# JacekNaruniec/LiveScan3D

Hardware: AMD Instinct MI355X
Metric: fused frames/s (N x 512x424 depth -> merged cloud) (higher is better)
Workload: dtype f32

## Files before the change

### livescan3d_amd/csrc/fusion.hip

```cpp


#include "fusion_shared.hpp"

namespace {

struct Iv { float lo, hi; };
__device__ __forceinline__ Iv iv_scale(Iv a, float c) { const float x = a.lo * c, y = a.hi * c; return c >= 0.0f ? Iv{x, y} : Iv{y, x}; }
__device__ __forceinline__ Iv iv_shift(Iv a, float c) { return Iv{a.lo + c, a.hi + c}; }
__device__ __forceinline__ Iv iv_sum(Iv a, Iv b) { return Iv{a.lo + b.lo, a.hi + b.hi}; }
__device__ __forceinline__ bool iv_finite(Iv a) { return isfinite(a.lo) && isfinite(a.hi); }

__device__ __forceinline__ float depth_to_metres1(float d)
{
    const f2 z = depth_to_metres2(f2{d, d});
    return z.x;
}

__device__ __forceinline__ int classify_range(int a, int b, float xfac, float yfac, const SensorParams &P, const float (&bx)[6])
{
    if (a == b) {
        f2 ox, oy, oz;
        unproject2(f2{(float)a, (float)a}, f2{xfac, xfac}, f2{yfac, yfac}, P, ox, oy, oz);
        const bool rejected = (ox.x < bx[0]) | (ox.x > bx[3]) | (oy.x < bx[1]) | (oy.x > bx[4]) | (oz.x < bx[2]) | (oz.x > bx[5]);
        return rejected ? 0 : 1;
// ... 116 lines not shown
#pragma unroll
        for (int i = 0; i < kTickGroup; i++) {
            const int wt = wave_count_thr(in[i], lo, cnt);
            if (lane == 0) s_cnt[wave][i] = wt;
        }
    } else {
        const SensorParams P = a.params[t.f];
        float xf[kPxPerLane], yf[kPxPerLane];
        tile_factors<VEC>(t, xf, yf);
#pragma unroll 1
        for (int i = 0; i < nt; i++) {
            Tile ti = t;
            ti.dptr = t.dptr + (long long)i * a.tick_depth_stride;
            Inputs ix;
            load_inputs<VEC, false>(ti, ix);
            bool keep[kPxPerLane];
            uint4 unused[kPxPerLane];
            compute_pixels<false>(a, P, ix, xf, yf, keep, unused);
            int wt = 0;
#pragma unroll
            for (int k = 0; k < kPxPerLane; k++) wt += __popcll(__ballot(keep[k]));
            if (lane == 0) s_cnt[wave][i] = wt;
        }
    }
    __syncthreads();
    if ((int)threadIdx.x < nt)
        a.tile_counts[(long long)(tick0 + threadIdx.x) * a.tiles_per_tick + tile] =
            s_cnt[0][threadIdx.x] + s_cnt[1][threadIdx.x] + s_cnt[2][threadIdx.x] + s_cnt[3][threadIdx.x];
}

constexpr unsigned long long kFlagAggregate = 1ull << 62;
constexpr unsigned long long kFlagPrefix = 2ull << 62;
constexpr int kSpinLimit = 1 << 20;

constexpr int kEpochShift = 34;
constexpr unsigned long long kTileAggregate = 1ull << 32, kTilePrefix = 2ull << 32;

__device__ __forceinline__ int tile_lookback(const FuseArgs &a, int tick, int tile, int tile_tot, int lane)
{
    unsigned long long *st = a.run_state + (long long)tick * a.tiles_per_tick;
    const unsigned long long tag = (unsigned long long)a.epoch << kEpochShift;
    if (lane == 0)
        __hip_atomic_store(&st[tile], tag | (tile == 0 ? kTilePrefix : kTileAggregate) | (unsigned int)tile_tot, __ATOMIC_RELAXED,
                           __HIP_MEMORY_SCOPE_AGENT);
    int acc = 0;
    int pos = tile - 1 - lane;
    bool done = tile == 0;
    int spins = 0;
    const bool near_polls = a.n_ticks > 1;
    while (!done) {
        unsigned long long w = tag | kTilePrefix;
        if (pos >= 0) {
            if (near_polls && (spins & 3) != 3) w = __hip_atomic_load(&st[pos], __ATOMIC_RELAXED, __HIP_MEMORY_SCOPE_WORKGROUP);
            else w = __hip_atomic_load(&st[pos], __ATOMIC_RELAXED, __HIP_MEMORY_SCOPE_AGENT);
        }
        bool again = false;
        const unsigned int flag = (w >> kEpochShift) == a.epoch ? (unsigned int)(w >> 32) & 3u : 0u;
        const unsigned long long pref = __ballot(flag == 2);
        const int first = pref ? __ffsll((long long)pref) - 1 : 63;
        const unsigned long long relevant = first >= 63 ? ~0ull : ((2ull << first) - 1ull);
        const bool poisoned = (__ballot(flag == 3) & relevant) != 0;
        if (poisoned || (__ballot(flag == 0) & relevant) != 0) {
            if (poisoned || ++spins > kSpinLimit) {
                if (lane == 0) {
                    atomicExch(a.error_flag, 1);
                    if (a.offsets_mirror) a.offsets_mirror[a.n_frames + 1] = 1;
                    __hip_atomic_store(&st[tile], tag | (3ull << 32), __ATOMIC_RELAXED, __HIP_MEMORY_SCOPE_AGENT);
                }
                return -1;
            }
            __builtin_amdgcn_s_sleep(1);
            again = true;
        } else {
            acc += wave_sum(lane <= first ? (int)(unsigned int)w : 0);
            if (pref) done = true;
        }
        if (!done && !again) pos -= 64;
    }
    if (lane == 0 && tile != 0)
        __hip_atomic_store(&st[tile], tag | kTilePrefix | (unsigned int)(acc + tile_tot), __ATOMIC_RELAXED, __HIP_MEMORY_SCOPE_AGENT);
    return acc;
}


template <int MODE, bool VEC, bool LAZY = false, bool HOST = false>
__global__ __launch_bounds__(kThreads) void fuse_kernel(const FuseArgs a)
{
    constexpr bool kWrite = MODE != 0;
    __shared__ uint4 stage[kWrite ? kStageSlots : 1];
    __shared__ int s_wave_tot[4];
    __shared__ int s_wave_next[4];
    __shared__ int s_base;
    const int lane = threadIdx.x & 63;
    const int wave = threadIdx.x >> 6;
    int tick = blockIdx.x / a.tiles_per_tick;
    int tile = blockIdx.x - tick * a.tiles_per_tick;
    if (kWrite && a.chunk > 0) {
        const int per_chunk = a.chunk * a.n_ticks;
        const int chunk = blockIdx.x / per_chunk;
        const int r = blockIdx.x - chunk * per_chunk;
        const int width = min(a.chunk, a.tiles_per_tick - chunk * a.chunk);
        tick = r / width;
        tile = chunk * a.chunk + (r - tick * width);
    }
    tile += a.tile0;
    if (MODE == 1 && a.reverse_ticks) tick = a.n_ticks - 1 - tick;
    const int lin = tick * a.tiles_per_tick + tile;

    const Tile t = locate(a, tick, tile);
    Inputs in;
    load_inputs<VEC, kWrite && !LAZY>(t, in);
    Inputs nx;
    if (MODE == 3) {
        Tile tn = t;
        tn.dptr = a.depth_next + tick * a.tick_depth_stride + t.pix_base;
        load_inputs<VEC, false>(tn, nx);
    }
    const SensorParams P = a.params[t.f];
    float xf[kPxPerLane], yf[kPxPerLane];
    tile_factors<VEC>(t, xf, yf);
    bool keep[kPxPerLane];
    uint4 vert[kPxPerLane];
    compute_pixels<kWrite>(a, P, in, xf, yf, keep, vert);
    if (kWrite && LAZY) {
        bool any = false;
#pragma unroll
        for (int k = 0; k < kPxPerLane; k++) any |= keep[k];
        if (any) {
            load_rgb<VEC>(t, in);
#pragma unroll
            for (int k = 0; k < kPxPerLane; k++) vert[k].x = rgba_of(in, k);
        }
    }
    if (MODE == 3) {
        int wt = 0;
        bool arithmetic = true;
        if (a.thr) {
            unsigned int lo[kPxPerLane], cnt[kPxPerLane];
            bool any_flagged;
            load_thresholds<VEC>(a, t, lo, cnt, any_flagged);
            arithmetic = any_flagged;
            if (!any_flagged) wt = wave_count_thr(nx, lo, cnt);
        }
        if (arithmetic) {
            bool keep_n[kPxPerLane];
            uint4 unused[kPxPerLane];
            compute_pixels<false>(a, P, nx, xf, yf, keep_n, unused);
#pragma unroll
            for (int k = 0; k < kPxPerLane; k++) wt += __popcll(__ballot(keep_n[k]));
        }
        if (lane == 0) s_wave_next[wave] = wt;
    }

    int below, wave_total;
    rank_from_masks(keep, below, wave_total);
    if (lane == 0) s_wave_tot[wave] = wave_total;
    int base = 0, counted = 0;
    if (MODE == 1 || MODE == 3) {
        base = a.tile_counts[lin];
        counted = (tile + 1 < a.tiles_per_tick ? a.tile_counts[lin + 1] : a.offsets[tick * (a.n_frames + 1) + a.n_frames]) - base;
    }
    __syncthreads();
    int wave_off = 0, tile_tot = 0;
#pragma unroll
    for (int i = 0; i < 4; i++) {
        const int v = s_wave_tot[i];
        if (i < wave) wave_off += v;
        tile_tot += v;
    }
    if (MODE == 0) {
        if (threadIdx.x == 0) a.tile_counts[lin] = tile_tot;
        return;
    }
    if (MODE == 3 && threadIdx.x == 0) a.tile_counts_next[lin] = s_wave_next[0] + s_wave_next[1] + s_wave_next[2] + s_wave_next[3];
    if (MODE == 4) {
        if (wave == 0) {
            const int b = tile_lookback(a, tick, tile, tile_tot, lane);
            if (lane == 0) s_base = b;
        }
        __syncthreads();
        base = s_base;
        if (base < 0) {
            if (threadIdx.x == 0 && tile == a.tiles_per_tick - 1) {
                a.offsets[tick * (a.n_frames + 1) + a.n_frames] = -1;
                if (a.offsets_mirror) a.offsets_mirror[a.n_frames] = -1;
            }
            return;
        }
        if (threadIdx.x == 0) {
            int *off = a.offsets + tick * (a.n_frames + 1);
            if (t.frame_start) off[t.f] = base;
            if (tile == a.tiles_per_tick - 1) off[a.n_frames] = base + tile_tot;
            if (a.offsets_mirror) {
                if (t.frame_start) a.offsets_mirror[t.f] = base;
                if (tile == a.tiles_per_tick - 1) a.offsets_mirror[a.n_frames] = base + tile_tot;
            }
            if (a.group_end_mirror && blockIdx.x == gridDim.x - 1) *a.group_end_mirror = base + tile_tot;
        }
    }
    if (MODE != 4 && tile_tot != counted) {
        if (threadIdx.x == 0) atomicExch(a.error_flag, 2);
        return;
    }
    if (VEC ? a.pm_first != nullptr : a.pixmap != nullptr) {
        const int p0 = t.px0 + threadIdx.x * kPxPerLane;
        if (p0 < t.npix) {
            int r = base + wave_off + below;
            if (VEC) {
                unsigned int m = 0;
#pragma unroll
                for (int k = 0; k < kPxPerLane; k++) m |= keep[k] ? (1u << k) : 0u;
                const long long g = (tick * a.tick_depth_stride + t.pix_base + p0) >> 3;
                a.pm_first[g] = r;
                a.pm_mask[g] = (unsigned char)m;
            } else {
                int *pm = a.pixmap + tick * a.tick_depth_stride + t.pix_base + p0;
#pragma unroll
                for (int k = 0; k < kPxPerLane; k++) {
                    if (p0 + k < t.npix) pm[k] = keep[k] ? r : -1;
                    r += keep[k] ? 1 : 0;
                }
            }
        }
    }
    stage_and_store(stage, keep, vert, wave_off + below, tile_tot, a.out + tick * a.tick_vert_stride + base, HOST || (MODE == 4 && a.host_out != 0));
}



template <bool VEC>
__global__ __launch_bounds__(kThreads) void run_kernel(const FuseArgs a)
{
    __shared__ uint4 stage[kStageSlots];
    __shared__ int s_wave_tot[4];
    __shared__ int s_run;
    __shared__ int s_base;
    const int lane = threadIdx.x & 63;
    const int wave = threadIdx.x >> 6;

    const int tick = blockIdx.x % a.n_ticks;
    if (threadIdx.x == 0) s_run = (int)atomicAdd(a.ticket + 32 * tick, 1u);
    __syncthreads();
    const int run = s_run;
    if (run >= a.runs_per_tick) return;
    const int t0 = run * a.tiles_per_run;
    const int t1 = min(t0 + a.tiles_per_run, a.tiles_per_tick);

    int wave_total = 0;
    {
        Tile t = locate(a, tick, t0);
        Inputs in;
        load_inputs<VEC, false>(t, in);
        for (int tile = t0; tile < t1; tile++) {
            Tile tn = t;
            Inputs nx = in;
            if (tile + 1 < t1) {
                tn = locate(a, tick, tile + 1);
                load_inputs<VEC, false>(tn, nx);
            }
            bool counted = false;
            if (a.thr) {
                unsigned int lo[kPxPerLane], cnt[kPxPerLane];
                bool any_flagged;
                load_thresholds<VEC>(a, t, lo, cnt, any_flagged);
                if (!any_flagged) {
                    wave_total += wave_count_thr(in, lo, cnt);
                    counted = true;
                }
            }
            if (!counted) {
                bool keep[kPxPerLane];
                uint4 unused[kPxPerLane];
                compute_tile<VEC, false>(a, t, in, keep, unused);
#pragma unroll
                for (int k = 0; k < kPxPerLane; k++) wave_total += __popcll(__ballot(keep[k]));
            }
            t = tn;
            in = nx;
        }
    }
    if (lane == 0) s_wave_tot[wave] = wave_total;
    __syncthreads();
    const int run_tot = s_wave_tot[0] + s_wave_tot[1] + s_wave_tot[2] + s_wave_tot[3];
// ... 30 lines not shown
            }
            const int v = (lane <= first) ? (int)(unsigned int)w : 0;
            acc += wave_sum(v);
            if (pref) done = true;
            else pos -= 64;
        }
        if (lane == 0) {
            if (run != 0) {
                const unsigned long long w = kFlagPrefix | (unsigned int)(acc + run_tot);
                __hip_atomic_store(&st[run], w, __ATOMIC_RELAXED, __HIP_MEMORY_SCOPE_AGENT);
            }
            s_base = acc;
        }
    }
    __syncthreads();
    int running = s_base;

    int *off = a.offsets + (long long)tick * (a.n_frames + 1);
    for (int tile = t0; tile < t1; tile++) {
        Tile tn = t;
        Inputs nx = in;
        if (tile + 1 < t1) {
            tn = locate(a, tick, tile + 1);
            load_inputs<VEC, true>(tn, nx);
        }
        bool keep[kPxPerLane];
        uint4 vert[kPxPerLane];
        compute_tile<VEC, true>(a, t, in, keep, vert);
        int below, wave_tot2;
        rank_from_masks(keep, below, wave_tot2);
        if (lane == 0) s_wave_tot[wave] = wave_tot2;
        __syncthreads();
        int wave_off = 0, tile_tot = 0;
#pragma unroll
        for (int i = 0; i < 4; i++) {
            const int v = s_wave_tot[i];
            if (i < wave) wave_off += v;
            tile_tot += v;
        }
        if (threadIdx.x == 0 && t.frame_start) off[t.f] = running;
        if (tile_tot > 0) {
            stage_and_store(stage, keep, vert, wave_off + below, tile_tot, a.out + tick * a.tick_vert_stride + running);
        } else {
            __syncthreads();
        }
        running += tile_tot;
        t = tn;
        in = nx;
    }
    if (threadIdx.x == 0 && t1 == a.tiles_per_tick) off[a.n_frames] = running;
}


__global__ __launch_bounds__(kThreads) void table_kernel(const FrameDesc *frames, const SensorParams *params, int n_frames, float *xtab,
                                                         float *ytab)
{
    const int f = blockIdx.y;
    if (f >= n_frames) return;
    const FrameDesc fd = frames[f];
    const SensorParams P = params[f];
    for (int i = blockIdx.x * kThreads + threadIdx.x; i < fd.w + fd.h; i += gridDim.x * kThreads) {
        if (i < fd.w) xtab[fd.xtab_off + i] = ((float)i - P.cx) / P.fx;
        else ytab[fd.ytab_off + (i - fd.w)] = (P.cy - (float)(i - fd.w)) / P.fy;
    }
}

}


extern "C" LsnFusion * lsnFusionCreate(int device, int n_ticks, int n_maps, const int *widths, const int *heights)
{
    return lsn::guarded("lsnFusionCreate", static_cast<LsnFusion *>(nullptr), [&]() -> LsnFusion * {
        lsn::clear_error();
        if (n_ticks <= 0 || n_maps <= 0 || !widths || !heights) {
            lsn::set_error("lsnFusionCreate: bad arguments (n_ticks=%d n_maps=%d)", n_ticks, n_maps);
            return nullptr;
        }
        LSN_HIP_NULL(hipSetDevice(device));
        LsnFusion *p = new (std::nothrow) LsnFusion();
        if (!p) return nullptr;
        p->device = device;
        if (const char *env = getenv("LSN_NO_THRESHOLDS")) p->thr_enabled = atoi(env) == 0;
        if (const char *env = getenv("LSN_LAZY_RGB")) p->lazy_rgb = atoi(env) != 0;

        p->n_ticks = n_ticks;
        p->n_maps = n_maps;
        std::vector<FrameDesc> fr(n_maps);
        std::vector<TileDesc> tf;
        long long doff = 0, coff = 0;
        int tiles = 0, xoff = 0, yoff = 0;
        bool vec = true;
        for (int i = 0; i < n_maps; i++) {
            if (widths[i] <= 0 || heights[i] <= 0 || (long long)widths[i] * heights[i] > (1ll << 30)) {
                lsn::set_error("lsnFusionCreate: bad frame size %dx%d", widths[i], heights[i]);
                delete p;
                return nullptr;
            }
            p->w.push_back(widths[i]);
            p->h.push_back(heights[i]);
            const int npix = widths[i] * heights[i];
            fr[i].w = widths[i];
            fr[i].h = heights[i];
            fr[i].npix = npix;
            fr[i].tile_start = tiles;
            p->tile_start.push_back(tiles);
            fr[i].depth_off = doff;
            fr[i].rgb_off = coff;
            fr[i].xtab_off = xoff;
            fr[i].ytab_off = yoff;
            fr[i].pad1 = 0;
            xoff += (widths[i] + 7) & ~7;
            yoff += heights[i];
            const int nt = (npix + kTile - 1) / kTile;
            fr[i].inv_w = 1.0f / (float)widths[i];
            for (int t = 0; t < nt; t++) {
                const long long px = (long long)t * kTile;
                TileDesc td;
                td.frame = i;
                td.y0 = (int)(px / widths[i]);
                td.x0 = (int)(px % widths[i]);
                td.pad = 0;
                tf.push_back(td);
            }
            tiles += nt;
            doff += npix;
            coff += 3ll * npix;
            if (widths[i] % 8 != 0) vec = false;
        }
        p->cap = doff;
        p->tick_depth_elems = doff;
        p->tick_rgb_bytes = coff;
        p->tiles_per_tick = tiles;
        p->one_tick_single_pass = n_ticks == 1 && tiles <= 2048;
        if (const char *env = getenv("LSN_ONE_TICK_SINGLE_PASS")) p->one_tick_single_pass = atoi(env) != 0;
        p->tile_start.push_back(tiles);
        p->vec_ok = vec;
        if (doff > 0x7FFFFFFFll) {
            lsn::set_error("lsnFusionCreate: a tick may not exceed 2^31-1 pixels (Mesh.nVertices is an int)");
            delete p;
            return nullptr;
        }
        if ((long long)tiles * n_ticks > 0x7FFFFFFFll) {
            lsn::set_error("lsnFusionCreate: too many tiles");
            delete p;
            return nullptr;
        }
        const size_t n_tiles_total = (size_t)tiles * n_ticks;
        if (p->frames.reserve(sizeof(FrameDesc) * n_maps) || p->tile_frame.reserve(sizeof(TileDesc) * tf.size()) ||
            p->params.reserve(sizeof(SensorParams) * n_maps) || p->tile_counts.reserve(sizeof(int) * n_tiles_total) ||
            p->tile_state.reserve(sizeof(unsigned long long) * n_tiles_total) || p->misc.reserve(128 * ((size_t)n_ticks + 1)) ||
            p->xtab.reserve(sizeof(float) * (size_t)(xoff + 8)) || p->ytab.reserve(sizeof(float) * (size_t)(yoff + 8))) {
            delete p;
            return nullptr;
        }
        if (hipMemset(p->misc.p, 0, 128 * ((size_t)n_ticks + 1)) != hipSuccess) {
            lsn::set_error("lsnFusionCreate: scratch initialisation failed");
            delete p;
            return nullptr;
        }
        if (hipMemcpy(p->frames.p, fr.data(), sizeof(FrameDesc) * n_maps, hipMemcpyHostToDevice) != hipSuccess ||
            hipMemcpy(p->tile_frame.p, tf.data(), sizeof(TileDesc) * tf.size(), hipMemcpyHostToDevice) != hipSuccess) {
            lsn::set_error("lsnFusionCreate: geometry upload failed");
            delete p;
            return nullptr;
        }
        return p;
    });
}

extern "C" void lsnFusionDestroy(LsnFusion *p)
{
    lsn::guarded_void("lsnFusionDestroy", [&]() {
        if (!p) return;
        (void)hipSetDevice(p->device);
        for (auto &e : p->events) {
            (void)hipEventDestroy(e.first);
            (void)hipEventDestroy(e.second);
        }
        p->rd.destroy_event();
        if (p->side) {
            (void)hipStreamSynchronize(p->side);
            (void)hipStreamDestroy(p->side);
            (void)hipEventDestroy(p->ev_counted);
            (void)hipEventDestroy(p->ev_written[0]);
            (void)hipEventDestroy(p->ev_written[1]);
        }
        delete p;
    });
}

extern "C" long long lsnFusionTickCapacity(const LsnFusion *p) { return p ? p->cap : 0; }

extern "C" int lsnPackSensorParams(const float *intr7, const float *wt12, float *out16)
{
    return lsn::guarded("lsnPackSensorParams", -1, [&]() {
        lsn::clear_error();
        if (!intr7 || !wt12 || !out16) {
            lsn::set_error("lsnPackSensorParams: null argument");
            return -1;
        }
        SensorParams s;
        pack_sensor_params(intr7, wt12, s);
        static_assert(sizeof(SensorParams) == 16 * sizeof(float), "SensorParams is 16 floats");
        memcpy(out16, &s, sizeof(s));
        return 0;
    });
}

extern "C" int lsnFusionSetParams(LsnFusion *p, const float *intr, const float *wt, const float *bounds6, void *stream)
{
    return lsn::guarded("lsnFusionSetParams", -1, [&]() {
        lsn::clear_error();
        if (!p || !intr || !wt || !bounds6) {
            lsn::set_error("lsnFusionSetParams: null argument");
            return -1;
        }
        LSN_HIP(hipSetDevice(p->device));
        {
            std::lock_guard<std::mutex> g(p->mu);
            if (p->params_set && p->last_intr.size() == 7 * (size_t)p->n_maps &&
                memcmp(p->last_intr.data(), intr, sizeof(float) * 7 * p->n_maps) == 0 &&
                memcmp(p->last_wt.data(), wt, sizeof(float) * 12 * p->n_maps) == 0 && memcmp(p->bounds, bounds6, sizeof(p->bounds)) == 0)
                return 0;
        }
        std::vector<SensorParams> sp(p->n_maps);
        for (int i = 0; i < p->n_maps; i++) pack_sensor_params(intr + 7 * i, wt + 12 * i, sp[i]);
        LSN_HIP(hipMemcpyAsync(p->params.p, sp.data(), sizeof(SensorParams) * p->n_maps, hipMemcpyHostToDevice,
                               lsn::as_stream(stream)));
        hipLaunchKernelGGL(table_kernel, dim3(8, (unsigned)p->n_maps), dim3(kThreads), 0, lsn::as_stream(stream), p->frames.as<FrameDesc>(),
                           p->params.as<SensorParams>(), p->n_maps, p->xtab.as<float>(), p->ytab.as<float>());
        LSN_HIP(hipGetLastError());
        LSN_HIP(hipStreamSynchronize(lsn::as_stream(stream)));
        std::lock_guard<std::mutex> g(p->mu);
// ... 21 lines not shown
}

extern "C" int lsnFusionSetPipelined(LsnFusion *p, int enable)
{
    return lsn::guarded("lsnFusionSetPipelined", -1, [&]() {
        lsn::clear_error();
        if (!p) return -1;
        std::lock_guard<std::mutex> g(p->mu);
        LSN_HIP(hipSetDevice(p->device));
        if (enable && !p->side) {
            if (p->tile_counts_b.reserve(sizeof(int) * (size_t)p->tiles_per_tick * p->n_ticks) ||
                p->offs_int.reserve(sizeof(int) * 2 * (size_t)p->n_ticks * (p->n_maps + 1)))
                return -1;
            LSN_HIP(hipStreamCreateWithFlags(&p->side, hipStreamNonBlocking));
            LSN_HIP(hipEventCreateWithFlags(&p->ev_counted, hipEventDisableTiming));
            LSN_HIP(hipEventCreateWithFlags(&p->ev_written[0], hipEventDisableTiming));
            LSN_HIP(hipEventCreateWithFlags(&p->ev_written[1], hipEventDisableTiming));
        }
        if (!enable && p->side) LSN_HIP(hipStreamSynchronize(p->side));
        p->pipelined = enable != 0;
        p->calls = 0;
        return 0;
    });
}

extern "C" int lsnFusionProfile(LsnFusion *p, int enable)
{
    return lsn::guarded("lsnFusionProfile", -1, [&]() {
        if (!p) return -1;
        p->profile = enable != 0;
        p->profile_every = enable > 1 ? enable : 1;
        p->profile_seq = 0;
        return 0;
    });
}

static int drain_events(LsnFusion *p)
{
    for (size_t i = 0; i < p->ev_used; i++) {
        float ms = 0;
        LSN_HIP(hipEventSynchronize(p->events[i].second));
        LSN_HIP(hipEventElapsedTime(&ms, p->events[i].first, p->events[i].second));
        p->acc_ms += ms;
        p->launches++;
    }
    p->ev_used = 0;
    return 0;
}

extern "C" int lsnFusionKernelStats(LsnFusion *p, double *avg_ms, long long *launches, char *name, int name_len, int reset)
{
    return lsn::guarded("lsnFusionKernelStats", -1, [&]() {
        lsn::clear_error();
        if (!p) return -1;
        std::lock_guard<std::mutex> g(p->mu);
        LSN_HIP(hipSetDevice(p->device));
        if (drain_events(p)) return -1;
        if (avg_ms) *avg_ms = p->launches ? p->acc_ms / (double)p->launches : 0.0;
        if (launches) *launches = p->launches;
        if (name && name_len > 0)
            snprintf(name, (size_t)name_len, "%s", p->timed_kernel ? p->timed_kernel : (p->mode == lsn::kPlanThreeLaunches ? "fuse_kernel<1>" : p->mode == lsn::kPlanSinglePass ? "fuse_kernel<4>" : "run_kernel"));
        if (reset) {
            p->acc_ms = 0;
            p->launches = 0;
        }
        return 0;
    });
}

void lsn::fill_args(LsnFusion *p, FuseArgs &a, const void *d_depth, const void *d_colors, void *d_vertices, int *d_offsets, bool with_pixmap)
{
    a.epoch = 0;
    a.chunk = 0;
    a.frames = p->frames.as<FrameDesc>();
    a.tiles = p->tile_frame.as<TileDesc>();
    a.params = p->params.as<SensorParams>();
    a.xtab = p->xtab.as<float>();
    a.ytab = p->ytab.as<float>();
    a.depth = static_cast<const unsigned short *>(d_depth);
    a.rgb = static_cast<const unsigned char *>(d_colors);
    a.out = static_cast<uint4 *>(d_vertices);
    a.tile_counts = p->tile_counts.as<int>();
    a.run_state = p->tile_state.as<unsigned long long>();
    a.error_flag = p->misc.as<int>();
    a.ticket = p->misc.as<unsigned int>() + 32;
    a.offsets = d_offsets;
    a.pixmap = with_pixmap ? p->pixmap.as<int>() : nullptr;
    a.pm_first = with_pixmap ? p->pm_first.as<int>() : nullptr;
    a.pm_mask = with_pixmap ? p->pm_mask.as<unsigned char>() : nullptr;
    a.n_frames = p->n_maps;
    a.tiles_per_tick = p->tiles_per_tick;
    a.n_ticks = p->n_ticks;
    {
        const long long total = (long long)p->tiles_per_tick * p->n_ticks;
        long long tpr = total / (6ll * 7 * 256);
        if (tpr < 1) tpr = 1;
        if (tpr > 8) tpr = 8;
        if (tpr > p->tiles_per_tick) tpr = p->tiles_per_tick;
        a.tiles_per_run = (int)tpr;
        a.runs_per_tick = (p->tiles_per_tick + a.tiles_per_run - 1) / a.tiles_per_run;
    }
    a.tick_depth_stride = p->tick_depth_elems;
    a.tick_rgb_stride = p->tick_rgb_bytes;
    a.tick_vert_stride = p->cap;
    a.minX = p->bounds[0]; a.minY = p->bounds[1]; a.minZ = p->bounds[2];
    a.maxX = p->bounds[3]; a.maxY = p->bounds[4]; a.maxZ = p->bounds[5];

    a.depth_next = nullptr;
    a.tile_counts_next = nullptr;
    a.thr = p->thr_valid ? p->thr.as<unsigned int>() : nullptr;
    a.tile0 = 0;
    a.reverse_ticks = 1;
    a.host_out = 0;
    a.offsets_mirror = nullptr;
    a.group_end_mirror = nullptr;
}

int lsn::ensure_thresholds(LsnFusion *p, hipStream_t s)
{
    if (!p->thr_enabled || p->thr_valid) return 0;
    if (++p->runs_with_params < 2) return 0;
    if (p->thr.reserve(sizeof(unsigned int) * (size_t)p->cap)) return -1;
    hipEvent_t e0, e1;
    LSN_HIP(hipEventCreate(&e0));
    LSN_HIP(hipEventCreate(&e1));
    LSN_HIP(hipEventRecord(e0, s));
    hipLaunchKernelGGL(thresh_kernel, dim3(256, (unsigned)p->n_maps), dim3(kThreads), 0, s, p->frames.as<FrameDesc>(), p->params.as<SensorParams>(),
                       p->n_maps, p->xtab.as<float>(), p->ytab.as<float>(), p->thr.as<unsigned int>(), p->bounds[0], p->bounds[1], p->bounds[2],
                       p->bounds[3], p->bounds[4], p->bounds[5]);
    LSN_HIP(hipGetLastError());
    LSN_HIP(hipEventRecord(e1, s));
    LSN_HIP(hipEventSynchronize(e1));
    (void)hipEventElapsedTime(&p->thr_build_ms, e0, e1);
    (void)hipEventDestroy(e0);
    (void)hipEventDestroy(e1);
    p->thr_valid = true;
    return 0;
}

template <int MODE, bool LAZY, bool HOST>
static void launch_fuse_as(bool vec, int grid, hipStream_t s, const FuseArgs &a)
{
    if (vec) hipLaunchKernelGGL((fuse_kernel<MODE, true, LAZY, HOST>), dim3(grid), dim3(kThreads), 0, s, a);
    else     hipLaunchKernelGGL((fuse_kernel<MODE, false, LAZY, HOST>), dim3(grid), dim3(kThreads), 0, s, a);
}

template <int MODE>
static void launch_fuse(bool vec, int grid, hipStream_t s, const FuseArgs &a, bool lazy_rgb = false, bool host_out = false)
{
    if constexpr (MODE == lsn::kPassWrite) {
        if (host_out) return launch_fuse_as<MODE, true, true>(vec, grid, s, a);
    }
    if constexpr (MODE == lsn::kPassWrite || MODE == lsn::kPassSingle) {
        if (lazy_rgb) return launch_fuse_as<MODE, true, false>(vec, grid, s, a);
    }
    launch_fuse_as<MODE, false, false>(vec, grid, s, a);
}

template <int kTickGroup>
static void launch_count_thr(bool vec, int grid, hipStream_t s, const FuseArgs &a)
{
    if (vec) hipLaunchKernelGGL((count_thr_kernel<true, kTickGroup>), dim3(grid), dim3(kThreads), 0, s, a);
    else     hipLaunchKernelGGL((count_thr_kernel<false, kTickGroup>), dim3(grid), dim3(kThreads), 0, s, a);
}

void lsn::count_and_scan(LsnFusion *p, bool vec, hipStream_t s, const FuseArgs &a, int *mirror)
{
    if (a.thr) {
        const int G = a.n_ticks >= 8 ? 8 : (a.n_ticks >= 4 ? 4 : 1);
        const int grid = p->tiles_per_tick * ((a.n_ticks + G - 1) / G);
        if (G == 8) launch_count_thr<8>(vec, grid, s, a);
        else if (G == 4) launch_count_thr<4>(vec, grid, s, a);
        else launch_count_thr<1>(vec, grid, s, a);
    } else {
        launch_fuse<lsn::kPassCount>(vec, p->tiles_per_tick * a.n_ticks, s, a);
    }
    hipLaunchKernelGGL(scan_kernel, dim3((unsigned)a.n_ticks), dim3(kScanThreads), 0, s, a.tile_counts, a.tiles_per_tick, a.frames, a.n_frames, a.offsets, mirror);
}

int lsn::next_event_pair(LsnFusion *p, hipEvent_t &e0, hipEvent_t &e1)
{
    if (p->ev_used == p->events.size()) {
        if (p->events.size() >= 4096) {
            if (drain_events(p)) return -1;
        } else {
            hipEvent_t x, y;
            LSN_HIP(hipEventCreate(&x));
            LSN_HIP(hipEventCreate(&y));
            p->events.emplace_back(x, y);
        }
    }
    e0 = p->events[p->ev_used].first;
    e1 = p->events[p->ev_used].second;
    p->ev_used++;
    return 0;
}

extern "C" int lsnFusionRun(LsnFusion *p, const void *d_depth, const void *d_colors, void *d_vertices, int *d_offsets,
                            void *stream)
{
    return lsn::guarded("lsnFusionRun", -1, [&]() {
        lsn::clear_error();
        return lsn::run_vertices(p, d_depth, d_colors, d_vertices, d_offsets, lsn::as_stream(stream));
    });
}

int lsn::run_vertices(LsnFusion *p, const void *d_depth, const void *d_colors, void *d_vertices, int *d_offsets, hipStream_t s)
{
    if (!p || !d_depth || !d_colors || !d_vertices || !d_offsets) {
        lsn::set_error("lsnFusionRun: null argument");
        return -1;
    }
    std::lock_guard<std::mutex> g(p->mu);
    return lsn::run_locked(p, d_depth, d_colors, d_vertices, d_offsets, s, false);
}

static int next_epoch(LsnFusion *p, hipStream_t s)
{
    if (p->epoch == 0 || p->epoch >= (1u << 30) - 1) {
        LSN_HIP(hipMemsetAsync(p->tile_state.p, 0, sizeof(unsigned long long) * (size_t)p->tiles_per_tick * p->n_ticks, s));
        p->epoch = 0;
    }
    ++p->epoch;
    return 0;
}


static int run_three_launches(LsnFusion *p, FuseArgs &a, bool vec, hipStream_t s, hipEvent_t e0, hipEvent_t e1)
{
    count_and_scan(p, vec, s, a);
    if (e0) LSN_HIP(hipEventRecord(e0, s));
    a.chunk = 0;
    launch_fuse<lsn::kPassWrite>(vec, p->tiles_per_tick * p->n_ticks, s, a, p->lazy_rgb);
    if (e1) LSN_HIP(hipEventRecord(e1, s));
    return 0;
}

static int run_pipelined(LsnFusion *p, FuseArgs &a, bool vec, hipStream_t s, hipEvent_t e0, hipEvent_t e1)
{
    const int b = (int)(p->calls & 1);
    const size_t off_elems = (size_t)p->n_ticks * (p->n_maps + 1);
    int *d_offsets = a.offsets, *off_int = p->offs_int.as<int>() + b * off_elems;
    a.tile_counts = b ? p->tile_counts_b.as<int>() : p->tile_counts.as<int>();
    if (p->calls >= 2) LSN_HIP(hipStreamWaitEvent(p->side, p->ev_written[b], 0));
    a.offsets = off_int;
    count_and_scan(p, vec, p->side, a);
    a.offsets = d_offsets;
    LSN_HIP(hipEventRecord(p->ev_counted, p->side));
    LSN_HIP(hipStreamWaitEvent(s, p->ev_counted, 0));
    LSN_HIP(hipMemcpyAsync(d_offsets, off_int, sizeof(int) * off_elems, hipMemcpyDeviceToDevice, s));
    if (e0) LSN_HIP(hipEventRecord(e0, s));
    launch_fuse<lsn::kPassWrite>(vec, p->tiles_per_tick * p->n_ticks, s, a);
    if (e1) LSN_HIP(hipEventRecord(e1, s));
    LSN_HIP(hipEventRecord(p->ev_written[b], s));
    p->calls++;
    return 0;
}

static int run_single_pass(LsnFusion *p, FuseArgs &a, bool vec, hipStream_t s, hipEvent_t e0, hipEvent_t e1)
{
    if (next_epoch(p, s)) return -1;
    a.epoch = p->epoch;
    constexpr int kFuseChunk = 16;
    a.chunk = kFuseChunk;
    if (e0) LSN_HIP(hipEventRecord(e0, s));
    launch_fuse<lsn::kPassSingle>(vec, p->tiles_per_tick * p->n_ticks, s, a, p->lazy_rgb);
    if (e1) LSN_HIP(hipEventRecord(e1, s));
    return 0;
}

static int run_lookback_runs(LsnFusion *p, FuseArgs &a, bool vec, hipStream_t s, hipEvent_t e0, hipEvent_t e1)
{
    LSN_HIP(hipMemsetAsync(p->tile_state.p, 0, sizeof(unsigned long long) * (size_t)p->tiles_per_tick * p->n_ticks, s));
    LSN_HIP(hipMemsetAsync(p->misc.as<char>() + 128, 0, 128 * (size_t)p->n_ticks, s));
    if (e0) LSN_HIP(hipEventRecord(e0, s));
    const int rgrid = a.runs_per_tick * p->n_ticks;
    if (vec) hipLaunchKernelGGL((run_kernel<true>), dim3(rgrid), dim3(kThreads), 0, s, a);
    else     hipLaunchKernelGGL((run_kernel<false>), dim3(rgrid), dim3(kThreads), 0, s, a);
    if (e1) LSN_HIP(hipEventRecord(e1, s));
    return 0;
}

enum class RunForm { ThreeLaunches, Pipelined, SinglePass, LookbackRuns };
static RunForm run_form(const LsnFusion *p, bool with_pixmap)
{
    switch (p->mode) {
    case lsn::kPlanThreeLaunches:
        if (p->pipelined) return with_pixmap ? RunForm::ThreeLaunches : RunForm::Pipelined;
        return p->n_ticks == 1 && p->one_tick_single_pass ? RunForm::SinglePass : RunForm::ThreeLaunches;
    case lsn::kPlanLookbackRuns:
        return with_pixmap ? RunForm::ThreeLaunches : RunForm::LookbackRuns;
    default:
        return with_pixmap ? RunForm::ThreeLaunches : RunForm::SinglePass;
    }
}

int lsn::run_locked(LsnFusion *p, const void *d_depth, const void *d_colors, void *d_vertices, int *d_offsets, hipStream_t s, bool with_pixmap)
{
    if (!p->params_set) {
        lsn::set_error("lsnFusionRun: lsnFusionSetParams has not been called");
        return -1;
    }
    if (((uintptr_t)d_vertices & 15) != 0) {
        lsn::set_error("lsnFusionRun: d_vertices must be 16-byte aligned");
        return -1;
    }
    LSN_HIP(hipSetDevice(p->device));
    if (ensure_thresholds(p, s)) return -1;
    FuseArgs a;
    fill_args(p, a, d_depth, d_colors, d_vertices, d_offsets, with_pixmap);
    const bool vec = wide_loads(p, d_depth, d_colors);

    hipEvent_t e0 = nullptr, e1 = nullptr;
    if (timed_launch(p) && next_event_pair(p, e0, e1)) return -1;

    const RunForm form = run_form(p, with_pixmap);
    if (p->mode == lsn::kPlanThreeLaunches) p->timed_kernel = form == RunForm::SinglePass ? "fuse_kernel<4>" : nullptr;
    int rc = -1;
    switch (form) {
    case RunForm::ThreeLaunches: rc = run_three_launches(p, a, vec, s, e0, e1); break;
    case RunForm::Pipelined:     rc = run_pipelined(p, a, vec, s, e0, e1); break;
    case RunForm::SinglePass:    rc = run_single_pass(p, a, vec, s, e0, e1); break;
    case RunForm::LookbackRuns:  rc = run_lookback_runs(p, a, vec, s, e0, e1); break;
    }
    if (rc) return -1;
    LSN_HIP(hipGetLastError());
    return 0;
}

int lsn::run_frames(LsnFusion *p, const void *d_depth, const void *d_colors, void *d_vertices, int *d_offsets, int f0, int f1, bool first_of_tick,
                    bool with_pixmap, int *offsets_mirror, int *group_end_mirror, bool host_out, hipStream_t s)
{
    if (!p || !d_depth || !d_colors || !d_vertices || !d_offsets || f0 < 0 || f1 > p->n_maps || f0 >= f1 || p->n_ticks != 1) {
        lsn::set_error("run_frames: bad arguments");
        return -1;
    }
    if (!p->params_set) {
        lsn::set_error("run_frames: lsnFusionSetParams has not been called");
        return -1;
    }
    std::lock_guard<std::mutex> g(p->mu);
    LSN_HIP(hipSetDevice(p->device));
    const bool vec = wide_loads(p, d_depth, d_colors);
    if (with_pixmap && reserve_pixmap(p, vec)) return -1;
    FuseArgs a;
    fill_args(p, a, d_depth, d_colors, d_vertices, d_offsets, with_pixmap);
    if (first_of_tick && next_epoch(p, s)) return -1;
    a.epoch = p->epoch;
    a.chunk = 0;
    a.tile0 = p->tile_start[f0];
    a.offsets_mirror = offsets_mirror;
    a.group_end_mirror = group_end_mirror;
    a.host_out = host_out ? 1 : 0;
    launch_fuse<lsn::kPassSingle>(vec, p->tile_start[f1] - p->tile_start[f0], s, a, p->lazy_rgb);
    LSN_HIP(hipGetLastError());
    return 0;
}

int lsn::run_count(LsnFusion *p, const void *d_depth, const void *d_colors, int *d_offsets, int *offsets_mirror, hipEvent_t counted, hipStream_t s)
{
    if (!p || !d_depth || !d_colors || !d_offsets || p->n_ticks != 1) {
        lsn::set_error("run_count: bad arguments");
        return -1;
    }
    if (!p->params_set) {
        lsn::set_error("run_count: lsnFusionSetParams has not been called");
        return -1;
    }
    std::lock_guard<std::mutex> g(p->mu);
    LSN_HIP(hipSetDevice(p->device));
    if (ensure_thresholds(p, s)) return -1;
    FuseArgs a;
    fill_args(p, a, d_depth, d_colors, nullptr, d_offsets, false);
    count_and_scan(p, wide_loads(p, d_depth, d_colors), s, a, offsets_mirror);
    LSN_HIP(hipGetLastError());
    if (counted) LSN_HIP(hipEventRecord(counted, s));
    return 0;
}

int lsn::run_write(LsnFusion *p, const void *d_depth, const void *d_colors, void *vertices, int *d_offsets, bool with_pixmap, bool host_out, hipStream_t s)
{
    if (!p || !d_depth || !d_colors || !vertices || !d_offsets || p->n_ticks != 1 || ((uintptr_t)vertices & 15) != 0) {
        lsn::set_error("run_write: bad arguments");
        return -1;
    }
    std::lock_guard<std::mutex> g(p->mu);
    LSN_HIP(hipSetDevice(p->device));
    const bool vec = wide_loads(p, d_depth, d_colors);
    if (with_pixmap && reserve_pixmap(p, vec)) return -1;
    FuseArgs a;
    fill_args(p, a, d_depth, d_colors, vertices, d_offsets, with_pixmap);
    launch_fuse<lsn::kPassWrite>(vec, p->tiles_per_tick, s, a, p->lazy_rgb, host_out);
    LSN_HIP(hipGetLastError());
    return 0;
}

extern "C" int lsnFusionRunStreamed(LsnFusion *p, const void *d_depth, const void *d_colors, void *d_vertices, int *d_offsets,
                                    const void *d_next_depth, void *stream)
{
    return lsn::guarded("lsnFusionRunStreamed", -1, [&]() {
        lsn::clear_error();
        if (!p || !d_depth || !d_colors || !d_vertices || !d_offsets) {
            lsn::set_error("lsnFusionRunStreamed: null argument");
            return -1;
        }
        if (!p->params_set) {
// ... 91 lines not shown
```

### livescan3d_amd/csrc/fusion_shared.hpp

```cpp
#pragma once

#include "lsn_common.hpp"
#include "wave_ops.hpp"

#include <cstdint>
#include <mutex>
#include <vector>

namespace lsn {

constexpr int kPlanThreeLaunches = 0;
constexpr int kPlanLookbackRuns = 1;
constexpr int kPlanSinglePass = 2;
constexpr int kPassCount = 0;
constexpr int kPassWrite = 1;
constexpr int kPassWriteCountNext = 3;
constexpr int kPassSingle = 4;

struct FrameDesc {
    int w, h, npix, tile_start;
    long long depth_off;
    long long rgb_off;
    int xtab_off, ytab_off;
    float inv_w;
    int pad1;
};

struct TileDesc {
    int frame;
    int x0, y0;
    int pad;
};

struct SensorParams {
    float cx, cy, fx, fy;
    float t0, t1, t2;
    float r00, r01, r02, r10, r11, r12, r20, r21, r22;
};

inline void pack_sensor_params(const float *ip, const float *tp, SensorParams &s)
{
    s.cx = ip[0]; s.cy = ip[1]; s.fx = ip[2]; s.fy = ip[3];
    s.t0 = tp[0]; s.t1 = tp[1]; s.t2 = tp[2];
    s.r00 = tp[3]; s.r01 = tp[4]; s.r02 = tp[5];
    s.r10 = tp[6]; s.r11 = tp[7]; s.r12 = tp[8];
    s.r20 = tp[9]; s.r21 = tp[10]; s.r22 = tp[11];
}

struct FuseArgs {
    const FrameDesc *frames;
    const TileDesc *tiles;
    const SensorParams *params;
    const float *xtab;
    const float *ytab;
    const unsigned short *depth;
    const unsigned char *rgb;
    uint4 *out;
    int *tile_counts;
    unsigned long long *run_state;
    unsigned int *ticket;
    int *offsets;
    int *pixmap;
    int *pm_first;
    unsigned char *pm_mask;
    const unsigned short *depth_next;
    int *tile_counts_next;
    int *error_flag;
    const unsigned int *thr;
    int n_frames;
    int tiles_per_tick;
    int n_ticks;
    int tiles_per_run;
    unsigned int epoch;
    int chunk;
    int reverse_ticks;
    int tile0;
    int host_out;
    int *group_end_mirror;
    int *offsets_mirror;
    int runs_per_tick;
    long long tick_depth_stride;
    long long tick_rgb_stride;
    long long tick_vert_stride;
    float minX, minY, minZ, maxX, maxY, maxZ;
};

struct TriArgs {
    const FrameDesc *frames;
    const TileDesc *tiles;
    const unsigned short *depth;
    const int *pixmap;
    const int *pm_first;
    const unsigned char *pm_mask;
    int *tri;
    int *tile_counts;
    unsigned int *codes;
    int tiles_per_tick;
    int win;
    int host_out;
    int index_base;
    long long tick_pix_stride;
    long long tick_tri_stride;
};

}
using lsn::FrameDesc;
using lsn::FuseArgs;
using lsn::TriArgs;
using lsn::SensorParams;
using lsn::pack_sensor_params;
using lsn::TileDesc;

namespace {

constexpr int kThreads = 256;
constexpr int kPxPerLane = 8;
constexpr int kTile = kThreads * kPxPerLane;
constexpr int kWin = 1152;
constexpr bool kNontemporalStores = true;



typedef float f2 __attribute__((ext_vector_type(2)));

__device__ __forceinline__ f2 depth_to_metres2(f2 d)
{
    const f2 r = {0x1.0624dep-10f, 0x1.0624dep-10f};
    const f2 k = {1000.0f, 1000.0f};
    const f2 q0 = d * r;
    const f2 e = __builtin_elementwise_fma(-q0, k, d);
    return __builtin_elementwise_fma(e, r, q0);
}

__device__ __forceinline__ void unproject2(f2 d, f2 xfac, f2 yfac, const SensorParams &P, f2 &ox, f2 &oy, f2 &oz)
{
    f2 Z = depth_to_metres2(d);
    f2 X = xfac * Z;
    f2 Y = yfac * Z;
    X = X + P.t0;
    Y = Y + P.t1;
    Z = Z + P.t2;
    ox = X * P.r00 + Y * P.r01 + Z * P.r02;
// ... 303 lines not shown
            round_tot += x;
        }
        pre += incl - t;
        if (whole) {
            reinterpret_cast<int4 *>(tc + i0)[0] = make_int4(pre + v[0], pre + v[1], pre + v[2], pre + v[3]);
            reinterpret_cast<int4 *>(tc + i0)[1] = make_int4(pre + v[4], pre + v[5], pre + v[6], pre + v[7]);
        } else {
#pragma unroll
            for (int k = 0; k < kScanItems; k++)
                if (i0 + k < tiles_per_tick) tc[i0 + k] = pre + v[k];
        }
        carry += round_tot;
        __syncthreads();
    }
    for (int f = threadIdx.x; f <= n_frames; f += kScanThreads) {
        const int v = f < n_frames ? tc[frames[f].tile_start] : carry;
        off[f] = v;
        if (mirror_row) mirror_row[f] = v;
    }
}

__attribute__((unused)) __global__ __launch_bounds__(kScanThreads) void scan_kernel(int *tile_counts, int tiles_per_tick, const FrameDesc *frames, int n_frames,
                                                        int *offsets, int *mirror)
{
    __shared__ int s_wave[kScanWaves];
    const int tick = blockIdx.x;
    scan_tick(tile_counts + (long long)tick * tiles_per_tick, tiles_per_tick, frames, n_frames, offsets + (long long)tick * (n_frames + 1),
                     mirror ? mirror + (long long)tick * (n_frames + 1) : nullptr, s_wave);
}


}


struct LsnFusion {
    int device = 0;
    int n_ticks = 0, n_maps = 0;
    std::vector<int> w, h;
    std::vector<int> tile_start;
    long long cap = 0;
    long long tick_depth_elems = 0, tick_rgb_bytes = 0;
    int tiles_per_tick = 0;
    bool vec_ok = false;
    bool params_set = false;
    int mode = lsn::kPlanThreeLaunches;
    unsigned int epoch = 0;
    float bounds[6] = {0, 0, 0, 0, 0, 0};
    lsn::DevBuf frames, tile_frame, params, tile_counts, tile_state, misc;
    lsn::DevBuf xtab, ytab;
    lsn::DevBuf pixmap, pm_first, pm_mask, tri_counts, tri_codes;
    bool pixmap_compact = false;
    lsn::RadialScratch rd;
    bool pipelined = false;
    hipStream_t side = nullptr;
    hipEvent_t ev_counted = nullptr, ev_written[2] = {nullptr, nullptr};
    lsn::DevBuf tile_counts_b, offs_int;
    unsigned long long calls = 0;
    const void *counted_for = nullptr;
    unsigned long long counted_gen = 0, params_gen = 1;
    int stream_half = 0;
    lsn::DevBuf thr;
    lsn::DevBuf ix_counts, ix_off, ix_pix2v, ix_v2pix, ix_conf, ix_ctile;
    bool ix_conf_ready = false;
    lsn::DevBuf ct_cov, ct_pairs, ct_blk, ct_stats, ct_samples, ct_xform;
    bool ct_ready = false;
    int ct_nblk = 0;
    lsn::DevBuf mg_toff, mg_depth0, mg_depth, mg_d2v, mg_assigned, mg_vconf, mg_proj, mg_zmax, mg_key, mg_mdepth, mg_mtag, mg_ero;
    bool mg_ready = false;
    lsn::DevBuf ol_key, ol_bucket, ol_chunk, ol_pts, ol_removed, ol_stats, ol_offs, ol_tab, ol_box, ol_frame;
    bool ol_ready = false;
    int ol_nb = 0, ol_nchunk = 0;
    lsn::DevBuf fl_tiles, fl_counts;
    std::vector<int> fl_tile_frame;
    bool fl_ready = false;
    int fl_tiles_per_tick = 0;
    int fl_last = 0;
    hipStream_t fl_stream = nullptr;
    lsn::RenderScratch rv;
    lsn::SimplifyScratch sp;
    lsn::NormalsScratch nm;
    bool thr_valid = false;
    bool thr_enabled = true;
    bool one_tick_single_pass = false;
    bool lazy_rgb = true;
    int runs_with_params = 0;
    std::vector<float> last_intr, last_wt;
    float thr_build_ms = 0;
    bool profile = false;
    int profile_every = 1;
    unsigned long long profile_seq = 0;
    std::vector<std::pair<hipEvent_t, hipEvent_t>> events;
    size_t ev_used = 0;
    double acc_ms = 0;
    long long launches = 0;
    const char *timed_kernel = nullptr;
    std::mutex mu;
};

namespace lsn {
inline bool wide_loads(const LsnFusion *p, const void *d_depth, const void *d_colors)
{
    return p->vec_ok && ((uintptr_t)d_depth & 15) == 0 && ((uintptr_t)d_colors & 7) == 0 && (p->tick_depth_elems % 8) == 0;
}
inline int reserve_pixmap(LsnFusion *p, bool vec)
{
    const size_t px = (size_t)p->cap * p->n_ticks;
    if (vec ? (p->pm_first.reserve(sizeof(int) * (px / 8 + 2)) || p->pm_mask.reserve(px / 8 + 2)) : p->pixmap.reserve(sizeof(int) * px)) return -1;
    p->pixmap_compact = vec;
    return 0;
}
void fill_args(LsnFusion *p, FuseArgs &a, const void *d_depth, const void *d_colors, void *d_vertices, int *d_offsets, bool with_pixmap);
int ensure_thresholds(LsnFusion *p, hipStream_t s);
void count_and_scan(LsnFusion *p, bool vec, hipStream_t s, const FuseArgs &a, int *mirror = nullptr);
int next_event_pair(LsnFusion *p, hipEvent_t &e0, hipEvent_t &e1);
inline bool timed_launch(LsnFusion *p) { return p->profile && (p->profile_every <= 1 || p->profile_seq++ % (unsigned long long)p->profile_every == 0); }
}
using lsn::ensure_thresholds;
using lsn::fill_args;
using lsn::count_and_scan;
using lsn::reserve_pixmap;
using lsn::wide_loads;
using lsn::next_event_pair;
using lsn::timed_launch;
```

Before: 220,500.

## Add single-launch frame-major fusion pass with per-frame decoupled lookback

Adds a new fuse pass (mode 5) that orders blocks frame-major across ticks and computes output offsets in one launch. Each block runs a decoupled lookback only within its own frame, using 128-wide wave loads, and chains to the previous frame through per-frame base words kept after the tile state. This replaces the three-launch count/scan/write path, removing extra launches and the second read of the depth data. In exchange it adds spin-wait dependencies between frames and a larger state buffer. The pass is chosen automatically only when there are many ticks and frames have at most 128 tiles, or when an environment variable forces it.

```diff
diff --git a/livescan3d_amd/csrc/fusion.hip b/livescan3d_amd/csrc/fusion.hip
--- a/livescan3d_amd/csrc/fusion.hip
+++ b/livescan3d_amd/csrc/fusion.hip
@@ -222,6 +222,59 @@
     return acc;
 }
 
+__device__ __forceinline__ unsigned int frame_word_flag(unsigned long long w, unsigned int epoch)
+{
+    return (unsigned int)(w >> kEpochShift) == epoch ? (unsigned int)(w >> 32) & 3u : 0u;
+}
+
+__device__ __forceinline__ int frame_lookback(const FuseArgs &a, int tick, int tile, const Tile &t, int tile_tot, int lane, unsigned long long wb)
+{
+    const int ftile = t.px0 / kTile, ftiles = (t.npix + kTile - 1) / kTile;
+    unsigned long long *st = a.run_state + (long long)tick * a.tiles_per_tick + (tile - ftile);
+    unsigned long long *bw = a.frame_base + (long long)tick * (a.n_frames + 1);
+    const unsigned long long tag = (unsigned long long)a.epoch << kEpochShift;
+    if (lane == 0) __hip_atomic_store(&st[ftile], tag | kTileAggregate | (unsigned int)tile_tot, __ATOMIC_RELAXED, __HIP_MEMORY_SCOPE_AGENT);
+    if (lane != 0 || t.f == 0) wb = tag | kTilePrefix;
+    int acc = 0, spins = 0;
+    bool bad = false;
+    int g = 0;
+    do {
+        const int pos0 = ftile - 1 - g - lane, pos1 = pos0 - 64;
+        unsigned long long w0 = tag | kTileAggregate, w1 = tag | kTileAggregate;
+        if (pos0 >= 0) w0 = __hip_atomic_load(&st[pos0], __ATOMIC_RELAXED, __HIP_MEMORY_SCOPE_AGENT);
+        if (pos1 >= 0) w1 = __hip_atomic_load(&st[pos1], __ATOMIC_RELAXED, __HIP_MEMORY_SCOPE_AGENT);
+        for (;;) {
+            const unsigned int f0 = frame_word_flag(w0, a.epoch), f1 = frame_word_flag(w1, a.epoch), fb = frame_word_flag(wb, a.epoch);
+            bad = __any(f0 == 3 || f1 == 3 || fb == 3);
+            if (bad || !__any(f0 == 0 || f1 == 0 || fb == 0)) break;
+            if (++spins > kSpinLimit) {
+                bad = true;
+                break;
+            }
+            __builtin_amdgcn_s_sleep(1);
+            if (f0 == 0) w0 = __hip_atomic_load(&st[pos0], __ATOMIC_RELAXED, __HIP_MEMORY_SCOPE_AGENT);
+            if (f1 == 0) w1 = __hip_atomic_load(&st[pos1], __ATOMIC_RELAXED, __HIP_MEMORY_SCOPE_AGENT);
+            if (fb == 0) wb = __hip_atomic_load(&bw[t.f], __ATOMIC_RELAXED, __HIP_MEMORY_SCOPE_AGENT);
+        }
+        if (bad) break;
+        acc += (int)(unsigned int)w0 + (int)(unsigned int)w1;
+        g += 128;
+    } while (g < ftile);
+    const bool frame_end = ftile == ftiles - 1;
+    if (bad) {
+        if (lane == 0) {
+            atomicExch(a.error_flag, 1);
+            __hip_atomic_store(&st[ftile], tag | (3ull << 32), __ATOMIC_RELAXED, __HIP_MEMORY_SCOPE_AGENT);
+            if (frame_end) __hip_atomic_store(&bw[t.f + 1], tag | (3ull << 32), __ATOMIC_RELAXED, __HIP_MEMORY_SCOPE_AGENT);
+        }
+        return -1;
+    }
+    const int pre = wave_sum(acc + (int)(unsigned int)wb);
+    if (lane == 0 && frame_end)
+        __hip_atomic_store(&bw[t.f + 1], tag | kTilePrefix | (unsigned int)(pre + tile_tot), __ATOMIC_RELAXED, __HIP_MEMORY_SCOPE_AGENT);
+    return pre;
+}
+
 
 template <int MODE, bool VEC, bool LAZY = false, bool HOST = false>
 __global__ __launch_bounds__(kThreads) void fuse_kernel(const FuseArgs a)
@@ -243,6 +296,13 @@
         tick = r / width;
         tile = chunk * a.chunk + (r - tick * width);
     }
+    if (MODE == lsn::kPassFrames) {
+        const FrameDesc fd = a.frames[a.tiles[blockIdx.x / a.n_ticks].frame];
+        const int ft = (fd.npix + kTile - 1) / kTile;
+        const int r = blockIdx.x - a.n_ticks * fd.tile_start;
+        tick = r / ft;
+        tile = fd.tile_start + (r - tick * ft);
+    }
     tile += a.tile0;
     if (MODE == 1 && a.reverse_ticks) tick = a.n_ticks - 1 - tick;
     const int lin = tick * a.tiles_per_tick + tile;
@@ -250,6 +310,9 @@
     const Tile t = locate(a, tick, tile);
     Inputs in;
     load_inputs<VEC, kWrite && !LAZY>(t, in);
+    unsigned long long base_word = 0;
+    if (MODE == lsn::kPassFrames && threadIdx.x == 0 && t.f > 0)
+        base_word = __hip_atomic_load(&a.frame_base[(long long)tick * (a.n_frames + 1) + t.f], __ATOMIC_RELAXED, __HIP_MEMORY_SCOPE_AGENT);
     Inputs nx;
     if (MODE == 3) {
         Tile tn = t;
@@ -313,9 +376,9 @@
         return;
     }
     if (MODE == 3 && threadIdx.x == 0) a.tile_counts_next[lin] = s_wave_next[0] + s_wave_next[1] + s_wave_next[2] + s_wave_next[3];
-    if (MODE == 4) {
+    if (MODE == 4 || MODE == lsn::kPassFrames) {
         if (wave == 0) {
-            const int b = tile_lookback(a, tick, tile, tile_tot, lane);
+            const int b = MODE == 4 ? tile_lookback(a, tick, tile, tile_tot, lane) : frame_lookback(a, tick, tile, t, tile_tot, lane, base_word);
             if (lane == 0) s_base = b;
         }
         __syncthreads();
@@ -338,7 +401,7 @@
             if (a.group_end_mirror && blockIdx.x == gridDim.x - 1) *a.group_end_mirror = base + tile_tot;
         }
     }
-    if (MODE != 4 && tile_tot != counted) {
+    if (MODE != 4 && MODE != lsn::kPassFrames && tile_tot != counted) {
         if (threadIdx.x == 0) atomicExch(a.error_flag, 2);
         return;
     }
@@ -535,6 +598,7 @@
         p->device = device;
         if (const char *env = getenv("LSN_NO_THRESHOLDS")) p->thr_enabled = atoi(env) == 0;
         if (const char *env = getenv("LSN_LAZY_RGB")) p->lazy_rgb = atoi(env) != 0;
+        if (const char *env = getenv("LSN_FRAMES_PASS")) p->frames_pass = atoi(env) != 0 ? 1 : 0;
 
         p->n_ticks = n_ticks;
         p->n_maps = n_maps;
@@ -575,6 +639,8 @@
                 td.pad = 0;
                 tf.push_back(td);
             }
+            if (i == 0 || nt < p->min_frame_tiles) p->min_frame_tiles = nt;
+            if (nt > p->max_frame_tiles) p->max_frame_tiles = nt;
             tiles += nt;
             doff += npix;
             coff += 3ll * npix;
@@ -601,7 +667,7 @@
         const size_t n_tiles_total = (size_t)tiles * n_ticks;
         if (p->frames.reserve(sizeof(FrameDesc) * n_maps) || p->tile_frame.reserve(sizeof(TileDesc) * tf.size()) ||
             p->params.reserve(sizeof(SensorParams) * n_maps) || p->tile_counts.reserve(sizeof(int) * n_tiles_total) ||
-            p->tile_state.reserve(sizeof(unsigned long long) * n_tiles_total) || p->misc.reserve(128 * ((size_t)n_ticks + 1)) ||
+            p->tile_state.reserve(sizeof(unsigned long long) * (n_tiles_total + (size_t)n_ticks * (n_maps + 1))) || p->misc.reserve(128 * ((size_t)n_ticks + 1)) ||
             p->xtab.reserve(sizeof(float) * (size_t)(xoff + 8)) || p->ytab.reserve(sizeof(float) * (size_t)(yoff + 8))) {
             delete p;
             return nullptr;
@@ -789,6 +855,7 @@
     a.out = static_cast<uint4 *>(d_vertices);
     a.tile_counts = p->tile_counts.as<int>();
     a.run_state = p->tile_state.as<unsigned long long>();
+    a.frame_base = a.run_state + (size_t)p->tiles_per_tick * p->n_ticks;
     a.error_flag = p->misc.as<int>();
     a.ticket = p->misc.as<unsigned int>() + 32;
     a.offsets = d_offsets;
@@ -858,7 +925,7 @@
     if constexpr (MODE == lsn::kPassWrite) {
         if (host_out) return launch_fuse_as<MODE, true, true>(vec, grid, s, a);
     }
-    if constexpr (MODE == lsn::kPassWrite || MODE == lsn::kPassSingle) {
+    if constexpr (MODE == lsn::kPassWrite || MODE == lsn::kPassSingle || MODE == lsn::kPassFrames) {
         if (lazy_rgb) return launch_fuse_as<MODE, true, false>(vec, grid, s, a);
     }
     launch_fuse_as<MODE, false, false>(vec, grid, s, a);
@@ -925,7 +992,7 @@
 static int next_epoch(LsnFusion *p, hipStream_t s)
 {
     if (p->epoch == 0 || p->epoch >= (1u << 30) - 1) {
-        LSN_HIP(hipMemsetAsync(p->tile_state.p, 0, sizeof(unsigned long long) * (size_t)p->tiles_per_tick * p->n_ticks, s));
+        LSN_HIP(hipMemsetAsync(p->tile_state.p, 0, p->tile_state.bytes, s));
         p->epoch = 0;
     }
     ++p->epoch;
@@ -976,6 +1043,17 @@
     return 0;
 }
 
+static int run_frames_pass(LsnFusion *p, FuseArgs &a, bool vec, hipStream_t s, hipEvent_t e0, hipEvent_t e1)
+{
+    if (next_epoch(p, s)) return -1;
+    a.epoch = p->epoch;
+    a.chunk = 0;
+    if (e0) LSN_HIP(hipEventRecord(e0, s));
+    launch_fuse<lsn::kPassFrames>(vec, p->tiles_per_tick * p->n_ticks, s, a, p->lazy_rgb);
+    if (e1) LSN_HIP(hipEventRecord(e1, s));
+    return 0;
+}
+
 static int run_lookback_runs(LsnFusion *p, FuseArgs &a, bool vec, hipStream_t s, hipEvent_t e0, hipEvent_t e1)
 {
     LSN_HIP(hipMemsetAsync(p->tile_state.p, 0, sizeof(unsigned long long) * (size_t)p->tiles_per_tick * p->n_ticks, s));
@@ -988,12 +1066,20 @@
     return 0;
 }
 
-enum class RunForm { ThreeLaunches, Pipelined, SinglePass, LookbackRuns };
+enum class RunForm { ThreeLaunches, Pipelined, SinglePass, LookbackRuns, FramesPass };
+constexpr int kFramesPassMaxTiles = 128;
+static bool frames_pass_chosen(const LsnFusion *p)
+{
+    if (p->frames_pass >= 0) return p->frames_pass != 0;
+    return (long long)p->n_ticks * p->min_frame_tiles >= 2ll * 7 * 256 && p->max_frame_tiles <= kFramesPassMaxTiles;
+}
+
 static RunForm run_form(const LsnFusion *p, bool with_pixmap)
 {
     switch (p->mode) {
     case lsn::kPlanThreeLaunches:
         if (p->pipelined) return with_pixmap ? RunForm::ThreeLaunches : RunForm::Pipelined;
+        if (!with_pixmap && frames_pass_chosen(p)) return RunForm::FramesPass;
         return p->n_ticks == 1 && p->one_tick_single_pass ? RunForm::SinglePass : RunForm::ThreeLaunches;
     case lsn::kPlanLookbackRuns:
         return with_pixmap ? RunForm::ThreeLaunches : RunForm::LookbackRuns;
@@ -1022,13 +1108,15 @@
     if (timed_launch(p) && next_event_pair(p, e0, e1)) return -1;
 
     const RunForm form = run_form(p, with_pixmap);
-    if (p->mode == lsn::kPlanThreeLaunches) p->timed_kernel = form == RunForm::SinglePass ? "fuse_kernel<4>" : nullptr;
+    if (p->mode == lsn::kPlanThreeLaunches)
+        p->timed_kernel = form == RunForm::SinglePass ? "fuse_kernel<4>" : form == RunForm::FramesPass ? "fuse_kernel<5>" : nullptr;
     int rc = -1;
     switch (form) {
     case RunForm::ThreeLaunches: rc = run_three_launches(p, a, vec, s, e0, e1); break;
     case RunForm::Pipelined:     rc = run_pipelined(p, a, vec, s, e0, e1); break;
     case RunForm::SinglePass:    rc = run_single_pass(p, a, vec, s, e0, e1); break;
     case RunForm::LookbackRuns:  rc = run_lookback_runs(p, a, vec, s, e0, e1); break;
+    case RunForm::FramesPass:    rc = run_frames_pass(p, a, vec, s, e0, e1); break;
     }
     if (rc) return -1;
     LSN_HIP(hipGetLastError());
diff --git a/livescan3d_amd/csrc/fusion_shared.hpp b/livescan3d_amd/csrc/fusion_shared.hpp
--- a/livescan3d_amd/csrc/fusion_shared.hpp
+++ b/livescan3d_amd/csrc/fusion_shared.hpp
@@ -16,6 +16,7 @@
 constexpr int kPassWrite = 1;
 constexpr int kPassWriteCountNext = 3;
 constexpr int kPassSingle = 4;
+constexpr int kPassFrames = 5;
 
 struct FrameDesc {
     int w, h, npix, tile_start;
@@ -58,6 +59,7 @@
     uint4 *out;
     int *tile_counts;
     unsigned long long *run_state;
+    unsigned long long *frame_base;
     unsigned int *ticket;
     int *offsets;
     int *pixmap;
@@ -527,6 +529,8 @@
     bool thr_valid = false;
     bool thr_enabled = true;
     bool one_tick_single_pass = false;
+    int frames_pass = -1;
+    int min_frame_tiles = 0, max_frame_tiles = 0;
     bool lazy_rgb = true;
     int runs_with_params = 0;
     std::vector<float> last_intr, last_wt;
```

New measurement: 134,000. -39.2%, worse.
